# CobaltCrabby/ray_tracer

Hardware: AMD Instinct MI355X
Metric: Mrays/s (reference-semantics closest-hit queries) at 1920x1080 Sponza (higher is better)
Workload: dtype f32; 1 GPU; sponza (synthetic-262267-tris), 1920x1080, 8 spp/step, bounceLimit 8, rows interleaved over 1 GPU(s), up to 10 steps in flight per rank (groups of 10+9+9+9); scene=sponza, assets=synthetic-262267-tris, width=1920, height=1080, frames_in_flight=10, pipeline=multi-kernel (k_trace_pw + k_shade per round)

## Files before the change

ray_tracer_amd/csrc/rt_kernels.hip.h:

```cpp
#pragma once

#include <hip/hip_runtime.h>
#include <stdint.h>

#include "rt_amd.h"
#include "rt_det_math.h"
#include "rt_probe.h"
#include "rt_ao_rays.h"
#include "scene_layout.h"
#include "launch_plan.h"
#include "temporal_motion.h"
#include "post_passes.h"

#ifndef RT_QUEUE_ORDER
#define RT_QUEUE_ORDER 0
#endif
#ifndef RT_TE_REG
#define RT_TE_REG 1
#endif
#ifndef RT_TE_REG_ALL
#define RT_TE_REG_ALL 1
#endif
#ifndef RT_SHADE_BLOCKS
#define RT_SHADE_BLOCKS 5
#endif
#ifndef RT_LEAF_PRELOAD
#define RT_LEAF_PRELOAD 1
#endif
#ifndef RT_OBJTREE
#define RT_OBJTREE 1
#endif
#ifndef RT_SHADE_IDENT
#define RT_SHADE_IDENT 1
#endif
#ifndef RT_FUSED_MAPS_BLOCKS
#define RT_FUSED_MAPS_BLOCKS 4
#endif
#define RT_HIT_NONE 0xffffffffu
#define RT_HIT_SPHERE 0x80000000u

struct DevScene {
    const float4* nodes;
    const float4* nodesPk;
    const uint32_t* leafFirst;
    const float4* triPos;
    const float4* triNrm;
    const float4* objInv;
    const float4* objFwd;
    const uint4* objMeta;
    const float4* objBox;
    const float4* mats;
    const float4* spheres;
    const uint32_t* sphereMat;
    uint32_t sphereCount, objectCount, materialCount, nodeCount, triCount;
    uint32_t hotNodes;
    uint32_t sphereTestMask;
    const float4* maskBox;
    const uint2* objSkipCost;
    uint32_t reachCount;
    const float4* objTree;
    const uint2* objCost;
    uint32_t objTreeOff[RT_OBJTREE_LEVELS + 1];
    uint32_t objTreeLevels;
    uint32_t maskBase;
    const uint2* emitTris;
    const float4* emitPre;
    uint32_t emitCount, emitSphereMask, emitMode;
    const uint32_t* texels;
    const uint4* texInfo;
    const float4* triUV;
    uint32_t texCount;
    const uint32_t* objAlpha;
    uint32_t mapFlags;
    float cullOriginLimit;
};

enum { RAY_MAIN = 0, RAY_NEE = 1, RAY_PROBE = 2 };
#define RAY_MAIN_BLANK 3u
__host__ __device__ __forceinline__ uint32_t ray_kind(uint32_t id) { return (id & 3u) == RAY_MAIN_BLANK ? (uint32_t)RAY_MAIN : (id & 3u); }

#define RT_STATE_F4_ARRAYS 15
struct PathState {
    float4* base;
    uint32_t pitch;
    uint32_t pitchStat;
    __host__ __device__ __forceinline__ float4* arr(uint32_t k) const { return base + (size_t)k * pitch; }
    __host__ __device__ __forceinline__ float4* rayO() const { return arr(0); }
    __host__ __device__ __forceinline__ float4* rayD() const { return arr(1); }
    __host__ __device__ __forceinline__ float4* auxO() const { return arr(2); }
    __host__ __device__ __forceinline__ float4* auxDL() const { return arr(3); }
    __host__ __device__ __forceinline__ float4* auxDC() const { return arr(4); }
    __host__ __device__ __forceinline__ float4* hit(uint32_t kind) const { return arr(5 + kind); }
    __host__ __device__ __forceinline__ float4* att() const { return arr(8); }
    __host__ __device__ __forceinline__ float4* total() const { return arr(9); }
    __host__ __device__ __forceinline__ float4* pendAlbedo() const { return arr(10); }
    __host__ __device__ __forceinline__ float4* accum() const { return arr(11); }
    __host__ __device__ __forceinline__ float4* camHit() const { return arr(12); }
    __host__ __device__ __forceinline__ float4* camDir() const { return arr(13); }
    __host__ __device__ __forceinline__ float4* pendMis() const { return arr(14); }
    __host__ __device__ __forceinline__ uint32_t* statBox() const { return (uint32_t*)arr(RT_STATE_F4_ARRAYS); }
    __host__ __device__ __forceinline__ uint32_t* statTri() const { return (uint32_t*)arr(RT_STATE_F4_ARRAYS) + pitchStat; }
};

struct Queues {
    uint32_t* active[2];
    uint32_t* rays[2];
    uint32_t* counts;
};

struct FrameParams {
    float camRot[16];
    float camPos[3];
    float planeWidth, planeHeight;
    float bottomLeft[3];
    uint32_t width, height, row0, rowStride, nRows, nPixels;
    uint32_t tiled;
    uint32_t startingSeed;
    uint32_t samples, bounceLimit;
    uint32_t progressive, frameCount;
    uint32_t camReuse;
    uint32_t nFrames;
    int32_t debug;
    uint32_t boxCap, triCap;
    EnvironmentData env;
    const uint32_t* sampleMap;
};

struct DevCounters {
    unsigned long long boxTests, triTests, raysTraced, raysHit, raysReference, paths, segments, emitterTests;
    unsigned long long skippedBoxTests;
};

#define RT_STAT_STRIPES 256u
struct ShadeStatStripe {
    unsigned long long raysReference, paths, segments, emitterTests;
    unsigned long long pad[12];
};

#define RT_AS_CONSTANT __attribute__((address_space(4)))
#define RT_AS_GLOBAL __attribute__((address_space(1)))
#define RT_AS_LDS __attribute__((address_space(3)))
typedef float rt_f4v __attribute__((ext_vector_type(4)));
typedef float rt_f2v __attribute__((ext_vector_type(2)));
template <typename T> __device__ __forceinline__ const T* rt_uniform(const T* p) { return (const T*)(const RT_AS_CONSTANT T*)(unsigned long long)p; }
template <typename T> __device__ __forceinline__ const T* rt_global(const T* p) { return (const T*)(const RT_AS_GLOBAL T*)(unsigned long long)p; }

__device__ __forceinline__ rt_vec3 f4xyz(float4 v) { return rt_v3(v.x, v.y, v.z); }
__device__ __forceinline__ float4 mk4(rt_vec3 v, float w) { return make_float4(v.x, v.y, v.z, w); }
__device__ __forceinline__ float4 mk4u(rt_vec3 v, uint32_t w) { return make_float4(v.x, v.y, v.z, __uint_as_float(w)); }

__device__ __forceinline__ rt_vec3 xform_dir_rows(float4 r0, float4 r1, float4 r2, rt_vec3 v) {
    return rt_v3((r0.x * v.x + r0.y * v.y) + r0.z * v.z, (r1.x * v.x + r1.y * v.y) + r1.z * v.z,
                 (r2.x * v.x + r2.y * v.y) + r2.z * v.z);
}
__device__ __forceinline__ rt_vec3 xform_point_rows(float4 r0, float4 r1, float4 r2, rt_vec3 v) {
    return rt_v3(((r0.x * v.x + r0.y * v.y) + r0.z * v.z) + r0.w, ((r1.x * v.x + r1.y * v.y) + r1.z * v.z) + r1.w,
                 ((r2.x * v.x + r2.y * v.y) + r2.z * v.z) + r2.w);
}

__device__ __forceinline__ uint32_t lane_id() { return __lane_id(); }
__device__ __forceinline__ uint32_t lanes_below(unsigned long long m) {
    return __builtin_amdgcn_mbcnt_hi((uint32_t)(m >> 32), __builtin_amdgcn_mbcnt_lo((uint32_t)m, 0u));
}
__device__ __forceinline__ unsigned long long wave_sum_u64(unsigned long long v) {
#pragma unroll
    for (int o = 32; o > 0; o >>= 1) v += __shfl_xor(v, o, RT_WAVE);
    return v;
}
__device__ __forceinline__ uint32_t wave_sum_u32(uint32_t v) {
#pragma unroll
    for (int o = 32; o > 0; o >>= 1) v += __shfl_xor(v, o, RT_WAVE);
    return v;
}

struct SphereHit { bool didHit, frontFace; float dst; };

__device__ __forceinline__ SphereHit sphere_intersect(float4 s, rt_vec3 ro, rt_vec3 rd) {
// ... 591 lines not shown
                    }
                    if (general) {
                        const float4 r0 = sc.objInv[3 * obj], r1 = sc.objInv[3 * obj + 1], r2 = sc.objInv[3 * obj + 2];
                        trd = xform_dir_rows(r0, r1, r2, wd);
                        wo = xform_point_rows(r0, r1, r2, wo);
                    } else {
                        trd = wd;
                    }
                    troXY = rt_f2{wo.x, wo.y};
                    invXY = rt_f2{1.f / trd.x, 1.f / trd.y};
                    zOI = rt_f2{wo.z, 1.f / trd.z};
                    atWorld = !general;
                    if (general) {
                        cur = nxW;
                        obj++;
                        fetch_next_meta();
                    } else {
                        cur = RT_CUR_NEED;
                    }
                }
            }
        }

        const unsigned long long tStep = STATS ? clock64() : 0ull;
        if (runI) {
            if (STATS) {
                wt.dbgRounds[2]++; wt.dbgLanes[2] += nI;
                wt.dbgWait[0] += __popcll(__ballot((int32_t)cur < 0 && cur < RT_CUR_LEAF_MAX));
                wt.dbgWait[1] += __popcll(__ballot(cur >= RT_CUR_LEAF_MAX && cur != RT_CUR_IDLE));
                wt.dbgWait[2] += __popcll(__ballot(cur == RT_CUR_IDLE));
            }
            if ((int32_t)cur >= 0) {
                float4 q0, q1, q2;
                float2 lk;
                if (HOT && cur < min(sc.hotNodes, 2u * (uint32_t)HOT)) {
                    const float4* ph = hotLds + 2 * cur;
                    q0 = ph[0]; q1 = ph[1]; q2 = ph[2];
                    lk = *(const float2*)(ph + 3);
                } else {
                    const float4* pr = sc.nodesPk + 2 * (size_t)cur;
                    q0 = pr[0]; q1 = pr[1]; q2 = pr[2];
                    lk = *(const float2*)(pr + 3);
                }
                if (STATS) RT_STAMP_AFTER_LOADS(wt.dbgLoad[2], tStep);
                float d1, d2;
                box_intersect_pair(q0, q1, q2, troXY, invXY, zOI, d1, d2);
                if (PIX) rayBox += 2; else wt.totBox += 2;
                const bool nearA = d1 <= d2;
                const float dNear = nearA ? d1 : d2, dFar = nearA ? d2 : d1;
                const uint32_t nW = __float_as_uint(nearA ? lk.x : lk.y), fW = __float_as_uint(nearA ? lk.y : lk.x);
                if (OVF) {
                    stack[min(sp, (uint32_t)STACK) * RT_WAVE] = fW;
                    if (sp >= (uint32_t)STACK && dFar < best) ovf[(sp - STACK) * ovfStride] = fW;
                } else {
                    stack[sp * RT_WAVE] = fW;
                }
                sp += (dFar < best) ? 1u : 0u;
                cur = (dNear < best) ? nW : RT_CUR_NEED;
            }
        }

        {
            const bool need = cur == RT_CUR_NEED;
            const bool has = sp > 0;
            uint32_t top;
            if (OVF) {
                top = stack[min((has ? sp : 1u) - 1u, (uint32_t)STACK) * RT_WAVE];
                if (need && sp > (uint32_t)STACK) top = ((const RT_AS_GLOBAL uint32_t*)ovf)[(sp - 1u - STACK) * ovfStride];
            } else {
                top = stack[((has ? sp : 1u) - 1u) * RT_WAVE];
            }
            const bool objLeft = obj < sc.objectCount;
            const bool ident = (nxFlags & RT_OBJ_IDENTITY) && plain;
            const uint32_t whenEmpty = objLeft ? (ident ? (atWorld ? nxW : RT_CUR_WORLD) : RT_CUR_SETUP) : RT_CUR_DONE;
            const bool enter = need && !has && objLeft && ident && atWorld;
            cur = need ? (has ? top : whenEmpty) : cur;
            sp -= (need && has) ? 1u : 0u;
            if (enter) {
                obj++;
                fetch_next_meta();
            }
            if (cur == RT_CUR_DONE) {
                const uint32_t slot = id >> 2, kind = LOCAL ? (id & 3u) : ray_kind(id);
                ps.hit(kind)[slot] = make_float4(best, __uint_as_float(bestObj), __uint_as_float(bestTri), 0.f);
                if (PIX && kind == RAY_MAIN) { ps.statBox()[slot] += rayBox; ps.statTri()[slot] += rayTri; }
                if (PIX) {
                    if (ta.perRayBox) { ta.perRayBox[qidx] = rayBox; ta.perRayTri[qidx] = rayTri; }
                    wt.totBox += rayBox; wt.totTri += rayTri;
                }
                wt.totHits += (bestObj != RT_HIT_NONE) ? 1u : 0u;
                cur = RT_CUR_IDLE;
            }
        }
        if (STATS) wt.dbgCycles[roundKind] += clock64() - tRound;
    }

}

__device__ __forceinline__ void fill_meta_lds(const DevScene& sc, uint2* s_meta) {
    if (threadIdx.x < RT_META_LDS) {
        uint2 m = make_uint2(0u, 0u);
        if (threadIdx.x < sc.objectCount) { const uint4 q = sc.objMeta[threadIdx.x]; m = make_uint2(q.x, q.w & 0xffu); }
        s_meta[threadIdx.x] = m;
    }
    __syncthreads();
}

template <int STACK, bool OVF, bool PIX, bool STATS, bool CULL, int HOT, bool ROOMY, bool ALPHA, int THREADS = RT_BLOCK>
__device__ __forceinline__ void trace_pw_block(const DevScene& sc, const PathState& ps, const TracePwArgs& ta) {
    __shared__ uint32_t s_stack[(THREADS / RT_WAVE) * (STACK + 1) * RT_WAVE];
    __shared__ uint2 s_meta[RT_META_LDS];
    __shared__ float4 s_hot[HOT ? 4 * HOT : 1];
    if (HOT) for (uint32_t k = threadIdx.x; k < 2u * min(sc.hotNodes, 2u * (uint32_t)HOT); k += THREADS) s_hot[k] = sc.nodesPk[k];
    fill_meta_lds(sc, s_meta);
    uint32_t* stack = s_stack + (threadIdx.x / RT_WAVE) * (STACK + 1) * RT_WAVE + (threadIdx.x & (RT_WAVE - 1));
    uint32_t* ovf = OVF ? ta.overflow + (size_t)blockIdx.x * THREADS + threadIdx.x : nullptr;
    const size_t ovfStride = (size_t)gridDim.x * THREADS;
    WaveTotals wt;
    const unsigned long long tStart = STATS ? wall_clock64() : 0ull;
    trace_wave<STACK, OVF, PIX, STATS, false, CULL, HOT, ROOMY, ALPHA, THREADS>(sc, ps, ta, stack, ovf, ovfStride, nullptr, *ta.count + (ta.countAux ? *ta.countAux + *ta.countAux2 : 0u), wt, s_meta, s_hot);

    const uint32_t skipTrips = STATS ? wave_sum_u32(wt.dbgWait[3]) : 0u;
    if (STATS && lane_id() == 0) {
        const size_t w = (size_t)blockIdx.x * (THREADS / RT_WAVE) + threadIdx.x / RT_WAVE;
        if (ta.waveTimes) {
            ta.waveTimes[2 * w] = tStart;
            ta.waveTimes[2 * w + 1] = wall_clock64();
        }
        for (int k = 0; k < 4; k++) {
            atomicAdd(&ta.phaseStats[k], (unsigned long long)wt.dbgRounds[k]);
            atomicAdd(&ta.phaseStats[4 + k], (unsigned long long)wt.dbgLanes[k]);
            atomicAdd(&ta.phaseStats[8 + k], wt.dbgCycles[k]);
            atomicAdd(&ta.phaseStats[16 + k], wt.dbgLoad[k]);
            if (k < 3) atomicAdd(&ta.phaseStats[12 + k], (unsigned long long)wt.dbgWait[k]);
            else atomicAdd(&ta.phaseStats[20], (unsigned long long)skipTrips);
        }
    }
    unsigned long long wb = wave_sum_u64(wt.totBox), wtri = wave_sum_u64(wt.totTri);
    uint32_t wr = wave_sum_u32(wt.totRays), wh = wave_sum_u32(wt.totHits);
    const unsigned long long wskip = CULL ? wave_sum_u64(wt.totSkipBox) : 0ull;
    if (lane_id() == 0 && wr) {
        if (CULL && wskip) atomicAdd(&ta.counters->skippedBoxTests, wskip);
        atomicAdd(&ta.counters->boxTests, wb);
        atomicAdd(&ta.counters->triTests, wtri);
        atomicAdd(&ta.counters->raysTraced, (unsigned long long)wr);
        atomicAdd(&ta.counters->raysHit, (unsigned long long)wh);
    }
}

template <int STACK, bool OVF, bool PIX, bool STATS, bool CULL, int HOT = 0, int BLOCKS = 6>
__global__ __launch_bounds__(RT_BLOCK, BLOCKS) void k_trace_pw(DevScene sc, PathState ps, TracePwArgs ta) {
    trace_pw_block<STACK, OVF, PIX, STATS, CULL, HOT, BLOCKS == 5 || (RT_TE_REG_ALL && !STATS), false>(sc, ps, ta);
}
template <int STACK, int HOT, int THREADS>
__global__ __launch_bounds__(THREADS, 6) void k_trace_pw_wide(DevScene sc, PathState ps, TracePwArgs ta) {
    trace_pw_block<STACK, false, false, false, false, HOT, true, false, THREADS>(sc, ps, ta);
}
template <bool PIX>
__global__ __launch_bounds__(RT_BLOCK, 4) void k_trace_pw_alpha(DevScene sc, PathState ps, TracePwArgs ta) {
    trace_pw_block<24, true, PIX, false, true, 0, true, true>(sc, ps, ta);
}

struct FullHit {
    rt_vec3 hitPoint, normal;
    uint32_t materialIndex;
    bool frontFace;
    float u, v;
};

__device__ __forceinline__ rt_vec3 albedo_texel(const DevScene& sc, uint32_t slot, uint32_t tri, uint32_t obj, rt_vec3 ro, rt_vec3 rd) {
    float bu, bv, bw;
    {
        const float4 i0 = rt_global(sc.objInv)[3 * obj], i1 = rt_global(sc.objInv)[3 * obj + 1], i2 = rt_global(sc.objInv)[3 * obj + 2];
        const float4 p0 = rt_global(sc.triPos)[3 * (size_t)tri], p1 = rt_global(sc.triPos)[3 * (size_t)tri + 1], p2 = rt_global(sc.triPos)[3 * (size_t)tri + 2];
        const TriHit h = tri_intersect(xform_point_rows(i0, i1, i2, ro), xform_dir_rows(i0, i1, i2, rd), f4xyz(p0), f4xyz(p1), f4xyz(p2), __float_as_uint(p0.w) != 0u);
        bu = h.u; bv = h.v; bw = h.w;
    }
    const float4 a = rt_global(sc.triUV)[2 * (size_t)tri], b = rt_global(sc.triUV)[2 * (size_t)tri + 1];
    float u = (bw * a.x + bu * a.z) + bv * b.x, v = (bw * a.y + bu * a.w) + bv * b.y;
    const bool e01 = a.x == a.z && a.y == a.w, e12 = a.z == b.x && a.w == b.y, e20 = b.x == a.x && b.y == a.y;
    if (e01 || e12 || e20) { u = 0.5f; v = 0.5f; }
    const uint4 ti = rt_global(sc.texInfo)[slot];
    const bool clampEdge = ((rt_global(sc.objMeta)[obj].w >> RT_OBJ_SAMPLER_SHIFT) & RT_OBJ_SAMPLER_MASK) == 1u;
    const uint32_t x = rt_tex_index(u, ti.y, clampEdge), y = rt_tex_index(1.f - v, ti.z, clampEdge);
    const uint32_t t = rt_global(sc.texels)[(size_t)ti.x + (size_t)y * ti.y + x];
    return rt_v3(rt_srgb8_to_linear(t & 0xffu), rt_srgb8_to_linear((t >> 8) & 0xffu), rt_srgb8_to_linear((t >> 16) & 0xffu));
}

template <bool MAPS = false>
__device__ __forceinline__ FullHit reconstruct_hit(const DevScene& sc, rt_vec3 ro, rt_vec3 rd, uint32_t obj, uint32_t tri) {
    FullHit f;
    f.u = 0.f; f.v = 0.f;
    if (obj & RT_HIT_SPHERE) {
        uint32_t i = obj & ~RT_HIT_SPHERE;
        float4 s = rt_global(sc.spheres)[i];
        SphereHit h = sphere_intersect(s, ro, rd);
        f.hitPoint = rt_add(ro, rt_scale(rd, h.dst));
        f.normal = rt_scale(rt_normalize(rt_sub(f.hitPoint, f4xyz(s))), h.frontFace ? 1.f : -1.f);
        f.materialIndex = rt_global(sc.sphereMat)[i];
        f.frontFace = h.frontFace;
        return f;
    }
    const uint4 meta = rt_global(sc.objMeta)[obj];
    const bool ident = RT_SHADE_IDENT && (meta.w & RT_OBJ_FWD_IDENTITY) && ray_is_plain(ro, rd);
    rt_vec3 trd = rd, tro = ro;
    if (!ident) {
        const float4* inv = rt_global(sc.objInv) + 3 * obj;
        const float4 i0 = inv[0], i1 = inv[1], i2 = inv[2];
        trd = xform_dir_rows(i0, i1, i2, rd);
        tro = xform_point_rows(i0, i1, i2, ro);
    }
    const float4* tp = rt_global(sc.triPos) + 3 * (size_t)tri;
    float4 a = tp[0], b = tp[1], c = tp[2];
    TriHit h = tri_intersect(tro, trd, f4xyz(a), f4xyz(b), f4xyz(c), __float_as_uint(a.w) != 0u);
    const float4* tn = rt_global(sc.triNrm) + 3 * (size_t)tri;
    rt_vec3 n0 = f4xyz(tn[0]), n1 = f4xyz(tn[1]), n2 = f4xyz(tn[2]);
    rt_vec3 ni = rt_add(rt_add(rt_scale(n0, h.w), rt_scale(n1, h.u)), rt_scale(n2, h.v));
    if (MAPS) {
        const HitUV q = hit_uv(sc, tri, h.u, h.v, h.w);
        f.u = q.u; f.v = q.v;
        const uint32_t bumpSlot = __float_as_uint(rt_global(sc.mats)[3 * meta.z + 2].w);
        if (bumpSlot < sc.texCount) {
            const bool clampEdge = ((meta.w >> RT_OBJ_SAMPLER_SHIFT) & RT_OBJ_SAMPLER_MASK) == 1u;
            const float h0 = rt_srgb8_to_linear(map_red8(sc, bumpSlot, clampEdge, q.u, q.v, false, false));
            const float hx = rt_srgb8_to_linear(map_red8(sc, bumpSlot, clampEdge, q.u, q.v, true, false)) - h0;
            const float hy = rt_srgb8_to_linear(map_red8(sc, bumpSlot, clampEdge, q.u, q.v, false, true)) - h0;
            ni = rt_bump_normal(ni, rt_sub(f4xyz(b), f4xyz(a)), rt_sub(f4xyz(c), f4xyz(a)), q.du1, q.dv1, q.du2, q.dv2, hx, hy);
        }
    }
    ni = rt_scale(ni, h.frontFace ? 1.f : -1.f);
    rt_vec3 op = rt_add(tro, rt_scale(trd, h.dst));
    if (ident && vec_is_plain(ni) && vec_is_plain(op)) {
        f.normal = rt_normalize(ni);
        f.hitPoint = op;
    } else {
        const float4* fwd = rt_global(sc.objFwd) + 3 * obj;
        const float4 m0 = fwd[0], m1 = fwd[1], m2 = fwd[2];
        f.normal = rt_normalize(xform_dir_rows(m0, m1, m2, ni));
        f.hitPoint = xform_point_rows(m0, m1, m2, op);
    }
    f.materialIndex = meta.z;
    f.frontFace = h.frontFace;
    return f;
}

__device__ __forceinline__ uint32_t hit_material(const DevScene& sc, uint32_t obj) {
    return (obj & RT_HIT_SPHERE) ? rt_global(sc.sphereMat)[obj & ~RT_HIT_SPHERE] : rt_global(sc.objMeta)[obj].z;
}

__device__ __forceinline__ float schlick(float cosine, float ri) {
    float r0 = (1.f - ri) / (1.f + ri);
    r0 = r0 * r0;
    return r0 + (1.f - r0) * rt_pow(1.f - cosine, 5.f);
}

__device__ __forceinline__ rt_vec3 environment_light(const EnvironmentData& env, rt_vec3 d) {
    if (!(env.lightDir[3] == 1.f)) return rt_v3(0.f, 0.f, 0.f);
    float skyT = rt_pow(rt_smoothstep(0.f, 0.4f, -d.y), 0.35f);
    rt_vec3 sky = rt_v3(rt_mix(env.horizonColor[0], env.zenithColor[0], skyT), rt_mix(env.horizonColor[1], env.zenithColor[1], skyT),
                        rt_mix(env.horizonColor[2], env.zenithColor[2], skyT));
    rt_vec3 negL = rt_v3(-env.lightDir[0], -env.lightDir[1], -env.lightDir[2]);
    float sun = rt_pow(rt_max(0.f, rt_dot(d, negL)), env.horizonColor[3]) * env.zenithColor[3];
    float g2s = rt_smoothstep(-0.01f, 0.f, -d.y);
    float sunMask = g2s >= 1.f ? 1.f : 0.f;
    float add = sun * sunMask;
    return rt_v3(rt_mix(env.groundColor[0], sky.x, g2s) + add, rt_mix(env.groundColor[1], sky.y, g2s) + add,
                 rt_mix(env.groundColor[2], sky.z, g2s) + add);
}

__device__ __forceinline__ float light_cos(rt_vec3 dir) { return rt_dot(rt_v3(0.f, -1.f, 0.f), dir); }
__device__ __forceinline__ float light_sample_pdf(const DevScene& sc, float t, uint32_t obj, float cosTheta) {
    if (obj == RT_HIT_NONE) return 0.f;
    uint32_t m = hit_material(sc, obj);
    if (rt_global(sc.mats)[3 * m + 1].w == 0.f) return 0.f;
    float sq = t * t;
    return sq / (cosTheta * 0.4444444f);
}

__device__ __forceinline__ rt_vec3 primary_dir(const FrameParams& fp, uint32_t gx, uint32_t gy) {
    float u = (float)gx / (float)fp.width;
    float v = (float)gy / (float)fp.height;
    rt_vec3 point = rt_add(rt_v3(fp.bottomLeft[0], fp.bottomLeft[1], fp.bottomLeft[2]),
                           rt_v3(fp.planeWidth * u, fp.planeHeight * v, 0.f));
    rt_vec3 dir = rt_normalize(point);
    return rt_xform_point(fp.camRot, dir);
}

__device__ __forceinline__ uint32_t slot_frame(const FrameParams& fp, uint32_t slot) { return (slot >> 6) % fp.nFrames; }
__device__ __forceinline__ uint32_t slot_in_tile(const FrameParams& fp, uint32_t slot) { return ((slot >> 6) / fp.nFrames << 6) | (slot & 63u); }
__device__ __forceinline__ uint32_t frame_slot(const FrameParams& fp, uint32_t frame, uint32_t tileSlot) {
    return ((tileSlot >> 6) * fp.nFrames + frame) * 64u + (tileSlot & 63u);
}

__device__ __forceinline__ void slot_to_pixel(const FrameParams& fp, uint32_t slot, uint32_t& gx, uint32_t& gy, uint32_t& k) {
    if (fp.nFrames > 1u) slot = slot_in_tile(fp, slot);
    const uint32_t tiledSlots = fp.tiled ? (fp.nRows & ~7u) * fp.width : 0u;
    if (slot < tiledSlots) {
        const uint32_t tile = slot >> 6, in = slot & 63u;
        const uint32_t tilesPerRow = fp.width >> 3;
        const uint32_t tyb = tile / tilesPerRow, txb = tile - tyb * tilesPerRow;
        gx = (txb << 3) + (in & 7u);
        k = (tyb << 3) + (in >> 3);
    } else {
        k = slot / fp.width;
        gx = slot - k * fp.width;
    }
    gy = fp.row0 + k * fp.rowStride;
}

__device__ __forceinline__ uint32_t pixel_samples(const FrameParams& fp, size_t px) {
    return fp.sampleMap ? min(rt_global(fp.sampleMap)[px], fp.samples) : fp.samples;
}

__device__ __forceinline__ uint32_t init_path(const DevScene& sc, const PathState& ps, const FrameParams& fp, uint32_t slot) {
    uint32_t gx, gy;
    uint32_t krow;
    slot_to_pixel(fp, slot, gx, gy, krow);
    const uint32_t samples = pixel_samples(fp, (size_t)krow * fp.width + gx);
    if (fp.sampleMap && samples == 0u) return 0u;
    ps.rayO()[slot] = make_float4(fp.camPos[0], fp.camPos[1], fp.camPos[2], 1.f);
    const rt_vec3 pd = primary_dir(fp, gx, gy);
    uint32_t startingSeed = fp.startingSeed;
    if (fp.nFrames > 1u) {
        uint32_t lol = fp.frameCount + slot_frame(fp, slot);
        startingSeed = (uint32_t)(rt_random(&lol) * 23892183.f);
    }
    ps.rayD()[slot] = mk4u(pd, gy * fp.width + gx + startingSeed);
    ps.camDir()[slot] = mk4u(pd, samples);
    ps.hit(RAY_MAIN)[slot] = sphere_seed(sc, rt_v3(fp.camPos[0], fp.camPos[1], fp.camPos[2]), pd);
    ps.att()[slot] = make_float4(1.f, 1.f, 1.f, __uint_as_float(0u));
    ps.total()[slot] = make_float4(0.f, 0.f, 0.f, __uint_as_float(0u));
    ps.accum()[slot] = make_float4(0.f, 0.f, 0.f, 0.f);
    ps.statBox()[slot] = 0;
    ps.statTri()[slot] = 0;
    return samples;
}

#define RT_QUEUE_HOLE 0xffffffffu
__global__ __launch_bounds__(RT_BLOCK) void k_raygen(DevScene sc, PathState ps, uint32_t* activeOut, uint32_t* raysOut, FrameParams fp,
                                                     uint32_t slotBegin, uint32_t slotEnd) {
    const uint32_t pos = blockIdx.x * RT_BLOCK + threadIdx.x;
    const uint32_t slot = slotBegin + pos;
    if (slot >= slotEnd) return;
    if (fp.nFrames > 1u && slot_in_tile(fp, slot) >= fp.nPixels) {
        activeOut[pos] = RT_QUEUE_HOLE;
        raysOut[pos] = RT_QUEUE_HOLE;
        return;
    }
    if (init_path(sc, ps, fp, slot) == 0u && fp.sampleMap) {
        activeOut[pos] = RT_QUEUE_HOLE;
        raysOut[pos] = RT_QUEUE_HOLE;
        return;
    }
    activeOut[pos] = slot;
    raysOut[pos] = slot << 2;
}

struct ShadeArgs {
    const uint32_t* inActive;
    const uint32_t* inCount;
    uint32_t* outActive;
    uint32_t* outRays;
    uint32_t* outActiveCount;
    uint32_t* outRayCount;
    ShadeStatStripe* stats;
    uint32_t* outAuxCount;
    uint32_t* outAuxCount2;
    uint32_t auxOffset;
};

template <bool MAPS = false, bool QUEUED = false, bool RAYS = false>
__device__ __forceinline__ void shade_path(const DevScene& sc, const PathState& ps, const FrameParams& fp, uint32_t slot, bool& alive,
                                           uint32_t& auxMask, uint32_t& refRays, uint32_t& nPaths, uint32_t& emitTests, bool withMask = true,
                                           const float* rayOrigins = nullptr) {
    bool wantAux = false;
    auxMask = 0;
    rt_vec3 auxOrigin = rt_v3(0, 0, 0), auxL = auxOrigin, auxC = auxOrigin;
    rt_vec3 auxAlbedo = auxOrigin;
    float auxNdotL = 0.f, auxCosPdfL = 0.f, auxCosPdfC = 0.f;
    float auxCosL = 0.f, auxCosC = 0.f;
    const float4 sO = ps.rayO()[slot], sD = ps.rayD()[slot], sA = ps.att()[slot], sT = ps.total()[slot];
    const float4 hM = (QUEUED && fp.camReuse && (__float_as_uint(sA.w) & 0x0fffffffu) == 0u && __float_as_uint(sT.w) != 0u) ? ps.camHit()[slot]
                                                                                                                        : ps.hit(RAY_MAIN)[slot];
    rt_vec3 ro = f4xyz(sO), rd = f4xyz(sD);
    rt_vec3 att = f4xyz(sA), total = f4xyz(sT);
    float misW = sO.w;
    uint32_t state = __float_as_uint(sD.w);
    uint32_t jraw = __float_as_uint(sA.w);
    uint32_t samplesDone = __float_as_uint(sT.w);
    uint32_t j = jraw & 0x0fffffffu;
    const bool pending = (jraw >> 31) != 0u;
    rt_vec3 direct = (jraw & 0x40000000u) ? rt_v3(-1.f, -1.f, -1.f) : rt_v3(0.f, 0.f, 0.f);
    bool specular = false;

    const uint32_t obj = __float_as_uint(hM.y);
    const uint32_t hitTriIdx = __float_as_uint(hM.z);
    refRays = 1;
    if (fp.camReuse && j == 0u && samplesDone == 0u) ps.camHit()[slot] = hM;

    bool done = false;
    bool zeroed = false;

    if (obj != RT_HIT_NONE) {
        if (pending) {
            float4 hL = make_float4(RT_MISS_DST, __uint_as_float(RT_HIT_NONE), 0.f, 0.f), hC = hL;
            if (!(jraw & 0x20000000u)) hL = ps.hit(RAY_NEE)[slot];
            if (!(jraw & 0x10000000u)) hC = ps.hit(RAY_PROBE)[slot];
            const float4 pM = ps.pendMis()[slot];
            float tL = hL.x, tC = hC.x;
            uint32_t oL = __float_as_uint(hL.y), oC = __float_as_uint(hC.y);
            uint32_t lm = (oL == RT_HIT_NONE) ? 0u : hit_material(sc, oL);
            float4 lmE = rt_global(sc.mats)[3 * lm + 1];
            float realLightPDF = light_sample_pdf(sc, tL, oL, pM.x);
            float cosinePDF = pM.z;
            float misWeight1 = realLightPDF * realLightPDF / (realLightPDF * realLightPDF + cosinePDF * cosinePDF);
            if (rt_isnan(misWeight1)) misWeight1 = 0.f;
            float lightPDF = light_sample_pdf(sc, tC, oC, pM.y);
            float realCosinePDF = pM.w;
            float misWeight2 = realCosinePDF * realCosinePDF / (lightPDF * lightPDF + realCosinePDF * realCosinePDF);
            if (rt_isnan(misWeight2)) misWeight2 = 0.f;
            const float4 pA = ps.pendAlbedo()[slot];
            rt_vec3 albedo = f4xyz(pA);
            rt_vec3 dl = rt_scale(rt_v3(lmE.x, lmE.y, lmE.z), lmE.w);
            float k = (realLightPDF == 0.f) ? 0.f : misWeight1 / realLightPDF;
            rt_vec3 f = rt_scale(rt_scale(rt_scale(albedo, RT_INV_PI), pA.w), k);
            direct = rt_mul(dl, f);
            misW = misWeight2;
        }

        FullHit hit = reconstruct_hit<MAPS>(sc, ro, rd, obj, hitTriIdx);
        const float4* mp = rt_global(sc.mats) + 3 * hit.materialIndex;
        float4 mA = mp[0], mE = mp[1], mI = mp[2];
        if (MAPS) {
            const uint32_t metalSlot = __float_as_uint(mI.z);
            if (metalSlot < sc.texCount && !(obj & RT_HIT_SPHERE))
                mA.w = rt_srgb8_to_linear(map_red8(sc, metalSlot, ((rt_global(sc.objMeta)[obj].w >> RT_OBJ_SAMPLER_SHIFT) & RT_OBJ_SAMPLER_MASK) == 1u, hit.u, hit.v, false, false));
        }

        rt_vec3 emission = rt_scale(rt_v3(mE.x, mE.y, mE.z), mE.w);
        emission = rt_v3(emission.x / misW, emission.y / misW, emission.z / misW);
        rt_vec3 finalLight = direct.x == -1.f ? emission : direct;
        total = rt_add(total, rt_mul(finalLight, att));
        if (j == 0) total = rt_add(total, emission);
        if (rt_isnan(total.x) || rt_isnan(total.y) || rt_isnan(total.z) || total.x < 0.f || total.y < 0.f || total.z < 0.f) {
            done = true;
            zeroed = true;
        } else {
            rt_vec3 sampledDir, radiance;
            float originSign = 1.f;
            bool diffuse = false;
            if (mA.w != 0.f) {
                sampledDir = rt_reflect(rd, hit.normal);
                radiance = rt_v3(1.f, 1.f, 1.f);
                specular = true;
                misW = 1.f;
            } else if (mI.x != -1.f) {
                float ior = !hit.frontFace ? mI.x : 1.f / mI.x;
                float cosine = rt_dot(rt_neg(rd), hit.normal);
                float sine = rt_sqrt(1.f - cosine * cosine);
                bool solution = (ior * sine) > 1.f;
                if (!solution) solution = schlick(cosine, ior) > rt_random(&state);
                sampledDir = solution ? rt_reflect(rd, hit.normal) : rt_refract(rd, hit.normal, ior);
                originSign = solution ? 1.f : rt_sign(rt_dot(hit.normal, rd));
                radiance = rt_v3(1.f, 1.f, 1.f);
                specular = true;
                misW = 1.f;
            } else {
                diffuse = true;
                refRays += 3;
                rt_vec3 albedo = rt_v3(mA.x, mA.y, mA.z);
                const uint32_t texSlot = __float_as_uint(mI.y);
                if (texSlot < sc.texCount && !(obj & RT_HIT_SPHERE)) albedo = rt_mul(albedo, albedo_texel(sc, texSlot, hitTriIdx, obj, ro, rd));
                rt_vec3 origin = rt_add(hit.hitPoint, rt_scale(hit.normal, 0.01f));
                float lx = rt_random(&state);
                float lz = rt_random(&state);
                rt_vec3 lp = rt_v3(rt_mix(-0.33333f, 0.33333f, lx), -1.5f, rt_mix(-0.33333f, 0.33333f, lz));
                rt_vec3 lightSample = rt_normalize(rt_sub(lp, origin));
                float r1 = rt_random(&state);
                float r2 = rt_random(&state);
                float phi = (2.f * RT_PI) * r1;
                float sqrtR2 = rt_sqrt(r2);
                float sn, cs;
                rt_sincos(phi, &sn, &cs);
                float x = cs * sqrtR2, y = sn * sqrtR2, z = rt_sqrt(1.f - r2);
                rt_vec3 axis = rt_abs(rt_dot(hit.normal, rt_v3(1.f, 0.f, 0.f))) < 1.f ? rt_v3(1.f, 0.f, 0.f) : rt_v3(0.f, 0.f, 1.f);
                rt_vec3 tt = rt_normalize(rt_cross(hit.normal, axis));
                rt_vec3 bb = rt_cross(hit.normal, tt);
                rt_vec3 cosineSample = rt_add(rt_add(rt_scale(tt, x), rt_scale(bb, y)), rt_scale(hit.normal, z));

                float realCosinePDF = rt_max(0.f, rt_dot(cosineSample, hit.normal) * RT_INV_PI);
                float nDotC = rt_dot(hit.normal, cosineSample);
                radiance = rt_scale(rt_scale(albedo, RT_INV_PI), nDotC);
                radiance = rt_v3(radiance.x / realCosinePDF, radiance.y / realCosinePDF, radiance.z / realCosinePDF);
                sampledDir = cosineSample;

                auxOrigin = origin; auxL = lightSample; auxC = cosineSample; auxAlbedo = albedo;
                auxCosL = light_cos(lightSample); auxCosC = light_cos(cosineSample);
                auxNdotL = rt_max(0.f, rt_dot(hit.normal, lightSample));
                auxCosPdfL = rt_max(0.f, rt_dot(lightSample, hit.normal) * RT_INV_PI);
                auxCosPdfC = realCosinePDF;
            }
            att = rt_mul(att, radiance);

            float rrProb = rt_max(rt_max(att.x, att.y), att.z);
            rrProb = rt_min(rrProb, 0.95f);
            rrProb = j <= 5 ? 1.f : rrProb;
            if (rt_random(&state) > rrProb) {
                done = true;
            } else {
                float invP = 1.f / rrProb;
                att = rt_scale(att, invP);
                ro = rt_add(hit.hitPoint, rt_scale(rt_scale(hit.normal, originSign), 0.00001f));
                rd = sampledDir;
                j++;
                if (j > fp.bounceLimit) done = true;
                else wantAux = diffuse;
            }
        }
    } else {
        total = rt_add(total, rt_mul(att, environment_light(fp.env, rd)));
        done = true;
    }

    if (done) {
        nPaths = 1;
        float4 acc = ps.accum()[slot];
        if (zeroed) total = rt_v3(0.f, 0.f, 0.f);
        const rt_vec3 sum = rt_add(f4xyz(acc), total);
        ps.accum()[slot] = mk4(sum, 0.f);
        samplesDone++;
        const float4 cD = ps.camDir()[slot];
        if (samplesDone < __float_as_uint(cD.w)) {
            if (RAYS) {
                const float* const o = rt_global(rayOrigins) + 3 * (size_t)slot;
                ro = rt_v3(o[0], o[1], o[2]);
            } else {
                ro = rt_v3(fp.camPos[0], fp.camPos[1], fp.camPos[2]);
            }
            rd = f4xyz(cD);
            att = rt_v3(1.f, 1.f, 1.f);
            total = rt_v3(0.f, 0.f, 0.f);
            specular = false;
            misW = 1.f;
            j = 0;
            alive = true;
            wantAux = false;
        }
    } else {
        alive = true;
    }

    if (alive) {
        if (done && fp.camReuse) {
            if (!QUEUED) ps.hit(RAY_MAIN)[slot] = ps.camHit()[slot];
            auxMask |= 4u;
        } else {
            const float4 seed = sphere_seed(sc, ro, rd, withMask);
            if (QUEUED && seed_is_blank(seed)) auxMask |= 8u;
            else ps.hit(RAY_MAIN)[slot] = seed;
        }
        if (wantAux) {
            float4 sL = sphere_seed(sc, auxOrigin, auxL, withMask), sC = sphere_seed(sc, auxOrigin, auxC, withMask);
            auxMask |= 3u;
            if (sc.emitMode) {
                float tL, tC;
                emitter_min_t2(sc, auxOrigin, auxL, auxC, tL, tC, emitTests);
                if (!(tL < RT_MISS_DST) || sL.x < tL) { sL.x = RT_MISS_DST; sL.y = __uint_as_float(RT_HIT_NONE); auxMask &= ~1u; }
                else sL.w = tL;
                if (!(tC < RT_MISS_DST) || sC.x < tC) { sC.x = RT_MISS_DST; sC.y = __uint_as_float(RT_HIT_NONE); auxMask &= ~2u; }
                else sC.w = tC;
            }
            const bool albedoFinite = !(rt_isnan(auxAlbedo.x) || rt_isnan(auxAlbedo.y) || rt_isnan(auxAlbedo.z) || rt_isinf(auxAlbedo.x) || rt_isinf(auxAlbedo.y) || rt_isinf(auxAlbedo.z));
            if ((auxMask & 3u) == 0u && albedoFinite) {
                float m2 = auxCosPdfC * auxCosPdfC / (0.f * 0.f + auxCosPdfC * auxCosPdfC);
                if (rt_isnan(m2)) m2 = 0.f;
                misW = m2;
                wantAux = false;
            } else {
                if (auxMask & 1u) ps.hit(RAY_NEE)[slot] = sL;
                if (auxMask & 2u) ps.hit(RAY_PROBE)[slot] = sC;
                if (auxMask & 3u) ps.auxO()[slot] = mk4(auxOrigin, 0.f);
                if (auxMask & 1u) ps.auxDL()[slot] = mk4(auxL, 0.f);
                if (auxMask & 2u) ps.auxDC()[slot] = mk4(auxC, 0.f);
                ps.pendAlbedo()[slot] = mk4(auxAlbedo, auxNdotL);
                ps.pendMis()[slot] = make_float4(auxCosL, auxCosC, auxCosPdfL, auxCosPdfC);
            }
        }
        const uint32_t answered = wantAux ? (((auxMask & 1u) ? 0u : 0x20000000u) | ((auxMask & 2u) ? 0u : 0x10000000u)) : 0u;
        ps.rayO()[slot] = mk4(ro, misW);
        ps.rayD()[slot] = mk4u(rd, state);
        ps.att()[slot] = mk4u(att, j | (wantAux ? 0x80000000u : 0u) | (specular ? 0x40000000u : 0u) | answered);
        const float4 nT = mk4u(total, samplesDone);
        if (!QUEUED || __float_as_uint(nT.x) != __float_as_uint(sT.x) || __float_as_uint(nT.y) != __float_as_uint(sT.y) ||
            __float_as_uint(nT.z) != __float_as_uint(sT.z) || __float_as_uint(nT.w) != __float_as_uint(sT.w))
            ps.total()[slot] = nT;
    }
}

template <bool MAPS, bool RAYS = false>
__device__ __forceinline__ void shade_block(const DevScene& sc, const PathState& ps, const ShadeArgs& sa, const FrameParams& fp,
                                            const float* rayOrigins = nullptr) {
    __shared__ uint32_t s_cnt[RT_BLOCK / RT_WAVE][8];
    __shared__ uint32_t s_base[4];
    const uint32_t n = *sa.inCount;
    if (blockIdx.x * RT_BLOCK >= n) return;
    const uint32_t gid = blockIdx.x * RT_BLOCK + threadIdx.x;
    const bool live = gid < n;

    bool alive = false;
    uint32_t auxMask = 0;
    uint32_t slot = 0;
    uint32_t refRays = 0, nPaths = 0, emitTests = 0;
    bool path = live;
    if (live) {
        slot = sa.inActive[gid];
        path = slot != 0xffffffffu;
        if (path) shade_path<MAPS, true, RAYS>(sc, ps, fp, slot, alive, auxMask, refRays, nPaths, emitTests, true, rayOrigins);
    }

    const unsigned long long mAlive = __ballot(alive), mM = __ballot(alive && !(auxMask & 4u));
    const unsigned long long mL = __ballot(alive && (auxMask & 1u)), mC = __ballot(alive && (auxMask & 2u));
    const uint32_t nAlive = __popcll(mAlive), nM = __popcll(mM), nL = __popcll(mL), nC = __popcll(mC);
    const uint32_t wRef = wave_sum_u32(refRays), wPaths = wave_sum_u32(nPaths), wSeg = wave_sum_u32(path ? 1u : 0u), wEmit = wave_sum_u32(emitTests);
    const uint32_t wv = threadIdx.x / RT_WAVE;
    if (lane_id() == 0) {
        s_cnt[wv][0] = nAlive; s_cnt[wv][1] = nM; s_cnt[wv][2] = wRef; s_cnt[wv][3] = wPaths; s_cnt[wv][4] = wSeg; s_cnt[wv][5] = wEmit; s_cnt[wv][6] = nL; s_cnt[wv][7] = nC;
    }
    __syncthreads();
    if (threadIdx.x == 0) {
        uint32_t tA = 0, tR = 0, tRef = 0, tP = 0, tS = 0, tE = 0, tX = 0, tY = 0;
        for (int w = 0; w < RT_BLOCK / RT_WAVE; w++) { tA += s_cnt[w][0]; tR += s_cnt[w][1]; tRef += s_cnt[w][2]; tP += s_cnt[w][3]; tS += s_cnt[w][4]; tE += s_cnt[w][5]; tX += s_cnt[w][6]; tY += s_cnt[w][7]; }
        s_base[0] = tA ? atomicAdd(sa.outActiveCount, tA) : 0u;
        s_base[1] = tR ? atomicAdd(sa.outRayCount, tR) : 0u;
        s_base[2] = tX ? atomicAdd(RT_QUEUE_ORDER ? sa.outAuxCount2 : sa.outAuxCount, tX) : 0u;
        s_base[3] = tY ? atomicAdd(RT_QUEUE_ORDER ? sa.outAuxCount : sa.outAuxCount2, tY) : 0u;
        ShadeStatStripe* const st = sa.stats + (blockIdx.x & (RT_STAT_STRIPES - 1u));
        atomicAdd(&st->raysReference, (unsigned long long)tRef);
        if (tP) atomicAdd(&st->paths, (unsigned long long)tP);
        atomicAdd(&st->segments, (unsigned long long)tS);
        if (tE) atomicAdd(&st->emitterTests, (unsigned long long)tE);
    }
    __syncthreads();
    if (alive) {
        uint32_t baseA = s_base[0], baseR = s_base[1];
        uint32_t baseX = (RT_QUEUE_ORDER ? 2u : 1u) * sa.auxOffset + s_base[2], baseY = (RT_QUEUE_ORDER ? 1u : 2u) * sa.auxOffset + s_base[3];
        for (uint32_t w = 0; w < wv; w++) { baseA += s_cnt[w][0]; baseR += s_cnt[w][1]; baseX += s_cnt[w][6]; baseY += s_cnt[w][7]; }
        sa.outActive[baseA + lanes_below(mAlive)] = slot;
        if (!(auxMask & 4u)) sa.outRays[baseR + lanes_below(mM)] = (slot << 2) | ((auxMask & 8u) ? RAY_MAIN_BLANK : (uint32_t)RAY_MAIN);
        if (auxMask & 1u) sa.outRays[baseX + lanes_below(mL)] = (slot << 2) | RAY_NEE;
        if (auxMask & 2u) sa.outRays[baseY + lanes_below(mC)] = (slot << 2) | RAY_PROBE;
    }
}

__global__ __launch_bounds__(RT_BLOCK, RT_SHADE_BLOCKS) void k_shade(DevScene sc, PathState ps, ShadeArgs sa, FrameParams fp) { shade_block<false>(sc, ps, sa, fp); }
__global__ __launch_bounds__(RT_BLOCK, RT_SHADE_BLOCKS) void k_shade_maps(DevScene sc, PathState ps, ShadeArgs sa, FrameParams fp) { shade_block<true>(sc, ps, sa, fp); }
__global__ __launch_bounds__(RT_BLOCK, RT_SHADE_BLOCKS) void k_shade_rays(DevScene sc, PathState ps, ShadeArgs sa, FrameParams fp, const float* origins, uint32_t first) {
    shade_block<false, true>(sc, ps, sa, fp, origins + 3 * (size_t)first);
}
__global__ __launch_bounds__(RT_BLOCK, RT_SHADE_BLOCKS) void k_shade_rays_maps(DevScene sc, PathState ps, ShadeArgs sa, FrameParams fp, const float* origins, uint32_t first) {
    shade_block<true, true>(sc, ps, sa, fp, origins + 3 * (size_t)first);
}

__device__ __forceinline__ rt_vec3 blend_frame(const FrameParams& fp, uint32_t samples, uint32_t frameCount, float4 oldc, float4 accum) {
    rt_vec3 out = f4xyz(accum);
    float fs = (float)samples;
    out = rt_v3(out.x / fs, out.y / fs, out.z / fs);
    float weight = 1.f / ((float)frameCount + 1.f);
    rt_vec3 blended = rt_add(rt_scale(rt_v3(oldc.x, oldc.y, oldc.z), 1.f - weight), rt_scale(out, weight));
    rt_vec3 fin = fp.progressive ? blended : out;
    if (rt_isnan(fin.x) || rt_isnan(fin.y) || rt_isnan(fin.z) || rt_isinf(fin.x) || rt_isinf(fin.y) || rt_isinf(fin.z))
        fin = rt_v3(1.f, 0.f, 1.f);
    return fin;
}

__device__ __forceinline__ void resolve_pixel(const PathState& ps, const FrameParams& fp, float4* rgba, uint32_t slot) {
    uint32_t gx, gy, krow;
    slot_to_pixel(fp, slot, gx, gy, krow);
    const size_t px = (size_t)krow * fp.width + gx;
    const uint32_t samples = pixel_samples(fp, px);
    if (fp.sampleMap && samples == 0u) return;
    rt_vec3 fin = blend_frame(fp, samples, fp.frameCount, rgba[px], ps.accum()[slot]);
    float s0 = (float)ps.statBox()[slot], s1 = (float)ps.statTri()[slot];
    float boxCap = (float)fp.boxCap, triCap = (float)fp.triCap;
    if (fp.debug == 0) {
        fin = s0 > boxCap ? rt_v3(1.f, 0.f, 0.f) : rt_v3(s0 / boxCap, s0 / boxCap, s0 / boxCap);
    } else if (fp.debug == 1) {
        fin = s1 > triCap ? rt_v3(1.f, 0.f, 0.f) : rt_v3(s1 / triCap, s1 / triCap, s1 / triCap);
    } else if (fp.debug == 2) {
        fin = rt_v3(s0 / boxCap, 0.f, s1 / triCap);
    }
    rgba[px] = make_float4(fin.x, fin.y, fin.z, 1.f);
}

__global__ __launch_bounds__(RT_BLOCK) void k_blend_frames(PathState ps, FrameParams fp, float4* rgba) {
    const uint32_t slot = blockIdx.x * RT_BLOCK + threadIdx.x;
    if (slot >= fp.nPixels) return;
    uint32_t gx, gy, krow;
    slot_to_pixel(fp, frame_slot(fp, 0u, slot), gx, gy, krow);
    const size_t px = (size_t)krow * fp.width + gx;
    const uint32_t samples = pixel_samples(fp, px);
    if (fp.sampleMap && samples == 0u) return;
    float4 c = rgba[px];
    for (uint32_t f = 0; f < fp.nFrames; f++) {
        const rt_vec3 fin = blend_frame(fp, samples, fp.frameCount + f, c, ps.accum()[frame_slot(fp, f, slot)]);
        c = make_float4(fin.x, fin.y, fin.z, 1.f);
    }
    rgba[px] = c;
}

__global__ __launch_bounds__(RT_BLOCK) void k_resolve(PathState ps, FrameParams fp, float4* rgba) {
    uint32_t slot = blockIdx.x * RT_BLOCK + threadIdx.x;
    if (slot >= fp.nPixels) return;
    resolve_pixel(ps, fp, rgba, slot);
}

struct FusedArgs {
    uint32_t* batchHead;
    float4* rgba;
    DevCounters* counters;
    uint32_t* overflow;
    uint32_t refill, wSetup, wLeaf, fastLanes;
    uint32_t batchPixels;
    uint32_t scatter;
    uint32_t fastShare;
    unsigned long long* waveTimes;
    uint32_t pixelRefill;
};

template <typename T>
__device__ __forceinline__ const T* opaque_kernarg() {
    unsigned long long v = (unsigned long long)__builtin_amdgcn_kernarg_segment_ptr();
    asm volatile("" : "+s"(v));
    return (const T*)(const RT_AS_CONSTANT T*)v;
}

struct FusedKernArgs {
    DevScene sc;
    PathState ps;
    FrameParams fp;
    FusedArgs fa;
};

template <int STACK, bool OVF, bool PIX, bool CULL>
__global__ __launch_bounds__(RT_BLOCK, 5) void k_render_fused(FusedKernArgs ka) {
    constexpr bool ALPHA = false, MAPS = false;
#include "rt_fused_body.hip.inc"
}
template <bool PIX>
// ... 579 lines not shown
```

Baseline: 5300 Mrays/s.

## Raise shade occupancy, cap wide-trace VGPRs, and trim shade register liveness

Raises the default shade kernel blocks-per-CU bound from 5 to 6. Caps the wide trace kernel at 36 VGPRs through an amdgpu_num_vgpr attribute. In shade_path it keeps only one dot product instead of several aux cosine/PDF values and computes the rest at store time, moves the rayD/total stores earlier, and pins the slot index in a VGPR, all to shorten live ranges. The aim is lower register pressure and higher occupancy, at the risk of spills from the tight VGPR cap and changed store ordering. The total-write skip now compares only xyz, with done forcing the write.

```diff
diff --git a/ray_tracer_amd/csrc/rt_kernels.hip.h b/ray_tracer_amd/csrc/rt_kernels.hip.h
--- a/ray_tracer_amd/csrc/rt_kernels.hip.h
+++ b/ray_tracer_amd/csrc/rt_kernels.hip.h
@@ -22,7 +22,7 @@
 #define RT_TE_REG_ALL 1
 #endif
 #ifndef RT_SHADE_BLOCKS
-#define RT_SHADE_BLOCKS 5
+#define RT_SHADE_BLOCKS 6
 #endif
 #ifndef RT_LEAF_PRELOAD
 #define RT_LEAF_PRELOAD 1
@@ -920,8 +920,9 @@
 __global__ __launch_bounds__(RT_BLOCK, BLOCKS) void k_trace_pw(DevScene sc, PathState ps, TracePwArgs ta) {
     trace_pw_block<STACK, OVF, PIX, STATS, CULL, HOT, BLOCKS == 5 || (RT_TE_REG_ALL && !STATS), false>(sc, ps, ta);
 }
+#define RT_WIDE_VGPR_REQUEST 36
 template <int STACK, int HOT, int THREADS>
-__global__ __launch_bounds__(THREADS, 6) void k_trace_pw_wide(DevScene sc, PathState ps, TracePwArgs ta) {
+__global__ __launch_bounds__(THREADS, 6) __attribute__((amdgpu_num_vgpr(RT_WIDE_VGPR_REQUEST))) void k_trace_pw_wide(DevScene sc, PathState ps, TracePwArgs ta) {
     trace_pw_block<STACK, false, false, false, false, HOT, true, false, THREADS>(sc, ps, ta);
 }
 template <bool PIX>
@@ -1145,8 +1146,7 @@
     auxMask = 0;
     rt_vec3 auxOrigin = rt_v3(0, 0, 0), auxL = auxOrigin, auxC = auxOrigin;
     rt_vec3 auxAlbedo = auxOrigin;
-    float auxNdotL = 0.f, auxCosPdfL = 0.f, auxCosPdfC = 0.f;
-    float auxCosL = 0.f, auxCosC = 0.f;
+    float auxDotL = 0.f, auxCosPdfC = 0.f;
     const float4 sO = ps.rayO()[slot], sD = ps.rayD()[slot], sA = ps.att()[slot], sT = ps.total()[slot];
     const float4 hM = (QUEUED && fp.camReuse && (__float_as_uint(sA.w) & 0x0fffffffu) == 0u && __float_as_uint(sT.w) != 0u) ? ps.camHit()[slot]
                                                                                                                         : ps.hit(RAY_MAIN)[slot];
@@ -1168,6 +1168,7 @@
 
     bool done = false;
     bool zeroed = false;
+    bool totalKept = false;
 
     if (obj != RT_HIT_NONE) {
         if (pending) {
@@ -1210,6 +1211,7 @@
         rt_vec3 finalLight = direct.x == -1.f ? emission : direct;
         total = rt_add(total, rt_mul(finalLight, att));
         if (j == 0) total = rt_add(total, emission);
+        totalKept = __float_as_uint(total.x) == __float_as_uint(sT.x) && __float_as_uint(total.y) == __float_as_uint(sT.y) && __float_as_uint(total.z) == __float_as_uint(sT.z);
         if (rt_isnan(total.x) || rt_isnan(total.y) || rt_isnan(total.z) || total.x < 0.f || total.y < 0.f || total.z < 0.f) {
             done = true;
             zeroed = true;
@@ -1263,9 +1265,7 @@
                 sampledDir = cosineSample;
 
                 auxOrigin = origin; auxL = lightSample; auxC = cosineSample; auxAlbedo = albedo;
-                auxCosL = light_cos(lightSample); auxCosC = light_cos(cosineSample);
-                auxNdotL = rt_max(0.f, rt_dot(hit.normal, lightSample));
-                auxCosPdfL = rt_max(0.f, rt_dot(lightSample, hit.normal) * RT_INV_PI);
+                auxDotL = rt_dot(hit.normal, lightSample);
                 auxCosPdfC = realCosinePDF;
             }
             att = rt_mul(att, radiance);
@@ -1318,15 +1318,19 @@
         alive = true;
     }
 
+    uint32_t wslot = slot;
+    if (QUEUED) asm volatile("" : "+v"(wslot));
     if (alive) {
         if (done && fp.camReuse) {
-            if (!QUEUED) ps.hit(RAY_MAIN)[slot] = ps.camHit()[slot];
+            if (!QUEUED) ps.hit(RAY_MAIN)[wslot] = ps.camHit()[wslot];
             auxMask |= 4u;
         } else {
             const float4 seed = sphere_seed(sc, ro, rd, withMask);
             if (QUEUED && seed_is_blank(seed)) auxMask |= 8u;
-            else ps.hit(RAY_MAIN)[slot] = seed;
-        }
+            else ps.hit(RAY_MAIN)[wslot] = seed;
+        }
+        ps.rayD()[wslot] = mk4u(rd, state);
+        if (!QUEUED || done || !totalKept) ps.total()[wslot] = mk4u(total, samplesDone);
         if (wantAux) {
             float4 sL = sphere_seed(sc, auxOrigin, auxL, withMask), sC = sphere_seed(sc, auxOrigin, auxC, withMask);
             auxMask |= 3u;
@@ -1345,23 +1349,18 @@
                 misW = m2;
                 wantAux = false;
             } else {
-                if (auxMask & 1u) ps.hit(RAY_NEE)[slot] = sL;
-                if (auxMask & 2u) ps.hit(RAY_PROBE)[slot] = sC;
-                if (auxMask & 3u) ps.auxO()[slot] = mk4(auxOrigin, 0.f);
-                if (auxMask & 1u) ps.auxDL()[slot] = mk4(auxL, 0.f);
-                if (auxMask & 2u) ps.auxDC()[slot] = mk4(auxC, 0.f);
-                ps.pendAlbedo()[slot] = mk4(auxAlbedo, auxNdotL);
-                ps.pendMis()[slot] = make_float4(auxCosL, auxCosC, auxCosPdfL, auxCosPdfC);
+                if (auxMask & 1u) ps.hit(RAY_NEE)[wslot] = sL;
+                if (auxMask & 2u) ps.hit(RAY_PROBE)[wslot] = sC;
+                if (auxMask & 3u) ps.auxO()[wslot] = mk4(auxOrigin, 0.f);
+                if (auxMask & 1u) ps.auxDL()[wslot] = mk4(auxL, 0.f);
+                if (auxMask & 2u) ps.auxDC()[wslot] = mk4(auxC, 0.f);
+                ps.pendAlbedo()[wslot] = mk4(auxAlbedo, rt_max(0.f, auxDotL));
+                ps.pendMis()[wslot] = make_float4(light_cos(auxL), light_cos(auxC), rt_max(0.f, auxDotL * RT_INV_PI), auxCosPdfC);
             }
         }
         const uint32_t answered = wantAux ? (((auxMask & 1u) ? 0u : 0x20000000u) | ((auxMask & 2u) ? 0u : 0x10000000u)) : 0u;
-        ps.rayO()[slot] = mk4(ro, misW);
-        ps.rayD()[slot] = mk4u(rd, state);
-        ps.att()[slot] = mk4u(att, j | (wantAux ? 0x80000000u : 0u) | (specular ? 0x40000000u : 0u) | answered);
-        const float4 nT = mk4u(total, samplesDone);
-        if (!QUEUED || __float_as_uint(nT.x) != __float_as_uint(sT.x) || __float_as_uint(nT.y) != __float_as_uint(sT.y) ||
-            __float_as_uint(nT.z) != __float_as_uint(sT.z) || __float_as_uint(nT.w) != __float_as_uint(sT.w))
-            ps.total()[slot] = nT;
+        ps.rayO()[wslot] = mk4(ro, misW);
+        ps.att()[wslot] = mk4u(att, j | (wantAux ? 0x80000000u : 0u) | (specular ? 0x40000000u : 0u) | answered);
     }
 }
 
```

After: 5508 Mrays/s, median of 6. 3.9% higher.
